# usnistgov/object-detection-yolov3

Measured on AMD Instinct MI355X. Metric: images/sec (train fwd+bwd) bs=8 416x416, higher is better.
Workload: dtype f32

## Files before the change

include/yolo3hip.h:

```cpp
#ifndef YOLO3HIP_H
#define YOLO3HIP_H

#include <math.h>
#include <stddef.h>
#include <stdint.h>

#ifdef __cplusplus
extern "C" {
#endif

#define Y3_OK 0
#define Y3_EINVAL (-1)
#define Y3_ELAUNCH (-2)

typedef void* y3_stream_t;

const char* y3_last_error(void);
int y3_debug_div(int x, int d);
int y3_version(void);

#define Y3_EPI_LRELU 1u
#define Y3_EPI_ACCUM 2u
#define Y3_CONV_X3 4u
int y3_x3_split_weights(const float* w, void* planes, int taps, int rows, int k_per_row, y3_stream_t stream);
// ... 1 lines not shown
int y3_x3_prepare_weights_batched(const float* params, float* params_t, void* planes, void* planes_t, const int* table_dev, int nlayers,
                                  int total_tiles, y3_stream_t stream);

typedef struct y3_tensor {
    float* ptr;
    int n, h, w, c;
    int ld;
} y3_tensor;

int y3_conv2d_fwd(const y3_tensor* src, const float* wt, const float* bias, int ksize, int stride,
                  const y3_tensor* dst, unsigned flags, float alpha,
                  const float* scale, const float* shift, const y3_tensor* resid,
                  float* stats, void* workspace, size_t workspace_bytes, y3_stream_t stream);
int y3_conv2d_stats_tiles(int m, int cin, int ksize, int cout);
size_t y3_conv2d_fwd_workspace(int m, int cin, int ksize, int cout);
int y3_conv2d_stats_tiles_x(int m, int cin, int ksize, int cout, unsigned flags);
size_t y3_conv2d_fwd_workspace_x(int m, int cin, int ksize, int cout, unsigned flags);
int y3_conv2d_x3_ok(int m, int c, int ntaps, int nout);
int y3_conv2d_dgrad_x3_ok(const y3_tensor* ddst, int ksize, int stride, const y3_tensor* dsrc);
size_t y3_conv2d_plan(int m, int cin, int ksize, int cout, int* out13);
size_t y3_conv2d_plan_x(int m, int cin, int ksize, int cout, unsigned flags, int* out13);

int y3_conv2d_dgrad(const y3_tensor* ddst, const float* wt_t, int ksize, int stride,
                    const y3_tensor* dsrc, unsigned flags, void* workspace, size_t workspace_bytes,
                    y3_stream_t stream);
size_t y3_conv2d_dgrad_workspace(const y3_tensor* ddst, int ksize, int stride, const y3_tensor* dsrc);
size_t y3_conv2d_dgrad_workspace_x(const y3_tensor* ddst, int ksize, int stride, const y3_tensor* dsrc, unsigned flags);
int y3_conv2d_dgrad_bn(const y3_tensor* ddst, const float* wt_t, int ksize, int stride, const y3_tensor* dsrc,
                       unsigned flags, const y3_tensor* bn_a, float* bn_partials,
                       void* workspace, size_t workspace_bytes, y3_stream_t stream);
int y3_conv2d_dgrad_bn_tiles(const y3_tensor* ddst, int ksize, int stride, const y3_tensor* dsrc);
int y3_conv2d_dgrad_bn_tiles_x(const y3_tensor* ddst, int ksize, int stride, const y3_tensor* dsrc, unsigned flags);
size_t y3_conv2d_dgrad_plan_x(const y3_tensor* ddst, int ksize, int stride, const y3_tensor* dsrc, unsigned flags, int* out51);

int y3_conv2d_wgrad(const y3_tensor* src, const y3_tensor* ddst, int ksize, int stride,
                    float* dw, void* workspace, size_t workspace_bytes, y3_stream_t stream);
size_t y3_conv2d_wgrad_workspace(const y3_tensor* src, const y3_tensor* ddst, int ksize, int stride);
int y3_conv2d_wgrad_x(const y3_tensor* src, const y3_tensor* ddst, int ksize, int stride,
                      float* dw, unsigned flags, void* workspace, size_t workspace_bytes, y3_stream_t stream);
size_t y3_conv2d_wgrad_workspace_x(const y3_tensor* src, const y3_tensor* ddst, int ksize, int stride, unsigned flags);
int y3_conv2d_wgrad_x3_ok(int m, int cin, int ksize, int cout);
size_t y3_conv2d_wgrad_plan(int m, int cin, int ksize, int cout, int* out8);
size_t y3_conv2d_wgrad_plan_x(int m, int cin, int ksize, int cout, unsigned flags, int* out8);

int y3_transpose_weights(const float* wt, float* wt_t, int taps, int cin, int cout, y3_stream_t stream);
int y3_transpose_weights_batched(const float* params, float* params_t, const int* table_dev, int nlayers,
                                 int total_tiles, y3_stream_t stream);

int y3_bn_stats_finalize(const float* stats, int tiles, int c, int count,
                         const float* gamma, const float* beta, float eps, float momentum,
                         float* moving_mean, float* moving_var,
                         float* save_mean, float* save_rstd, float* scale, float* shift,
                         y3_stream_t stream);
int y3_bn_fold_inference(const float* gamma, const float* beta, const float* moving_mean,
                         const float* moving_var, float eps, int c, float* scale, float* shift,
                         y3_stream_t stream);
int y3_bn_fold_inference_batched(const float* params, const float* moving, float* chan, const int* table_dev,
                                 int nlayers, float eps, y3_stream_t stream);
int y3_bn_apply(const y3_tensor* a, const float* scale, const float* shift, const y3_tensor* resid,
                const y3_tensor* y, y3_stream_t stream);
int y3_bn_bwd_stats(const y3_tensor* dy, const y3_tensor* a, const y3_tensor* dres, int dres_accumulate,
                    const float* gamma, const float* save_mean, const float* save_rstd, float alpha,
                    float* dgamma, float* dbeta, float* dbias, float* coef,
                    void* workspace, size_t workspace_bytes, y3_stream_t stream);
size_t y3_bn_bwd_workspace(int m, int c);
int y3_bn_bwd_apply(const y3_tensor* dy, const y3_tensor* a, const float* coef, float alpha,
// ... 277 lines not shown
```

object-detection-yolov3_amd/csrc/conv.hip:

```cpp
#include <stdlib.h>

#include <type_traits>
#include <utility>

#include "common.h"
#include "conv_plan.h"

template <int BM, int BN, int WM, int WN, int BK>
__global__ __launch_bounds__(64 * WM * WN) void conv_igemm_kernel(const ConvArgs p) {
    constexpr int THREADS = 64 * WM * WN;
    constexpr int LDA = BK + 4;
    constexpr int TM = BM / WM, TN = BN / WN, MB = TM / 32, NB = TN / 32;
    constexpr int KV = BK / 4;
    constexpr int A_TOTAL = BM * KV, A_LOADS = (A_TOTAL + THREADS - 1) / THREADS;
    constexpr int BN4 = BN / 4;
    constexpr int B_TOTAL = BK * BN4, B_LOADS = (B_TOTAL + THREADS - 1) / THREADS;
    static_assert(THREADS % KV == 0 && TM % 32 == 0 && TN % 32 == 0, "tile shape");

    __shared__ __attribute__((aligned(16))) float As[2][BM * LDA];
    __shared__ __attribute__((aligned(16))) float Bs[2][BK * BN];
    __shared__ float red[2][WM][BN];

    const int tid = threadIdx.x, lane = tid & 63, wave = tid >> 6;
    const int l31 = lane & 31, lh = lane >> 5;
// ... 1075 lines not shown
        a.nb_fast = a.nbn;
        a.dv_nb = y3_make_div(a.nbn);
        set_split(a, q);
        a.sk_slab0 = 0;
        const bool split = q.s0 > 1;
        a.tickets = split ? (int*)workspace + tick : nullptr;
        a.slab = split ? (float*)((char*)workspace + Y3_WS_HEADER) + slab_floats : nullptr;
        if (split) {
            tick += q.tiles;
            slab_floats += (size_t)q.tiles * q.s0 * t.bm * t.bn;
        }
        a.bn_row0 = rows;
        rows += a.nbm;
        m.first[c] = first;
        first += q.tiles * q.s0;
    }
    for (int c = ncls; c <= 4; ++c) m.first[c] = first;
    const bool bns = cls[0].bn_a != nullptr;
    if (cls[0].x3) {
        if (pl.ws > 0)
            if (int e = check_tickets("conv2d_dgrad (stride 2, x3)", workspace, st)) return e;
        if (!y3_x3_multi_launch(m, t.bn, bns, first, st)) {
            y3_set_error("conv2d_dgrad: no merged x3 kernel for tile %dx%d", t.bm, t.bn);
            return Y3_EINVAL;
        }
    } else if (!(bns ? launch_fast_multi<true>(t, m, first, st) : launch_fast_multi<false>(t, m, first, st))) {
        y3_set_error("conv2d_dgrad: no merged kernel for tile %dx%d", t.bm, t.bn);
        return Y3_EINVAL;
    }
    Y3_CHECK_LAUNCH("conv_igemm_fast_multi");
    return Y3_OK;
}

static int issue_dgrad(DgradDesc& d, const y3_tensor* ddst, const float* wt_t, const y3_tensor* dsrc, const y3_tensor* bn_a, float* bn_partials,
                       void* workspace, size_t workspace_bytes, hipStream_t st) {
    for (int c = 0; c < d.ncls; ++c) {
        ConvArgs& p = d.cls[c];
        p.src = ddst->ptr;
        p.wt = wt_t;
        p.dst = dsrc->ptr;
        if (bn_a) {
            p.bn_a = bn_a->ptr;
            p.bn_a_ld = bn_a->ld;
            p.bn_part = bn_partials;
        }
    }
    if (d.how == DGRAD_MERGED_F32 || d.how == DGRAD_MERGED_X3) return launch_dgrad_multi(d.cls, d.ncls, d.multi, workspace, workspace_bytes, st);
    for (int c = 0; c < d.ncls; ++c)
        if (int e = launch_igemm(d.cls[c], d.g[c], workspace, workspace_bytes, st)) return e;
    return Y3_OK;
}

static int check_dgrad_args(const y3_tensor* ddst, const float* wt_t, int ksize, int stride, const y3_tensor* dsrc, unsigned flags) {
    if (int e = check_tensor(ddst, "conv2d_dgrad ddst")) return e;
    if (int e = check_tensor(dsrc, "conv2d_dgrad dsrc")) return e;
    Y3_CHECK_ARG(wt_t, "conv2d_dgrad: null weights");
    Y3_CHECK_ARG((flags & ~(Y3_EPI_ACCUM | Y3_CONV_X3)) == 0, "conv2d_dgrad: only Y3_EPI_ACCUM and Y3_CONV_X3 allowed");
    Y3_CHECK_ARG(!(flags & Y3_CONV_X3) || dgrad_x3(flags, ddst, ksize, stride, dsrc), "conv2d_dgrad: Y3_CONV_X3 does not take this shape (ask y3_conv2d_dgrad_x3_ok())");
    return Y3_OK;
}
extern "C" int y3_conv2d_dgrad(const y3_tensor* ddst, const float* wt_t, int ksize, int stride, const y3_tensor* dsrc, unsigned flags,
                               void* workspace, size_t workspace_bytes, y3_stream_t stream) {
    if (int e = check_dgrad_args(ddst, wt_t, ksize, stride, dsrc, flags)) return e;
    DgradDesc d;
    if (int e = describe_dgrad(ddst, ksize, stride, dsrc, flags, &d)) return e;
    return issue_dgrad(d, ddst, wt_t, dsrc, nullptr, nullptr, workspace, workspace_bytes, (hipStream_t)stream);
}
extern "C" int y3_conv2d_dgrad_bn(const y3_tensor* ddst, const float* wt_t, int ksize, int stride, const y3_tensor* dsrc, unsigned flags,
                                  const y3_tensor* bn_a, float* bn_partials, void* workspace, size_t workspace_bytes, y3_stream_t stream) {
    if (int e = check_tensor(bn_a, "conv2d_dgrad_bn bn_a")) return e;
    Y3_CHECK_ARG(bn_partials, "conv2d_dgrad_bn: null partials");
    Y3_CHECK_ARG(dsrc && bn_a->n == dsrc->n && bn_a->h == dsrc->h && bn_a->w == dsrc->w && bn_a->c == dsrc->c, "conv2d_dgrad_bn: bn_a must have dsrc's geometry");
    Y3_CHECK_ARG((long long)bn_a->n * bn_a->h * bn_a->w * bn_a->ld * 4 < 0x7fffffffLL, "conv2d_dgrad_bn: bn_a of 2 GiB or more");
    DgradDesc d;
    Y3_CHECK_ARG(ddst && describe_dgrad(ddst, ksize, stride, dsrc, flags, &d) == Y3_OK && d.rows > 0, "conv2d_dgrad_bn: shape does not qualify (y3_conv2d_dgrad_bn_tiles() == 0)");
    if (int e = check_dgrad_args(ddst, wt_t, ksize, stride, dsrc, flags)) return e;
    return issue_dgrad(d, ddst, wt_t, dsrc, bn_a, bn_partials, workspace, workspace_bytes, (hipStream_t)stream);
}

extern "C" int y3_conv2d_wgrad(const y3_tensor* src, const y3_tensor* ddst, int ksize, int stride, float* dw, void* workspace,
                               size_t workspace_bytes, y3_stream_t stream) {
    return y3_conv2d_wgrad_x(src, ddst, ksize, stride, dw, 0u, workspace, workspace_bytes, stream);
}

extern "C" int y3_conv2d_wgrad_x(const y3_tensor* src, const y3_tensor* ddst, int ksize, int stride, float* dw, unsigned flags, void* workspace,
                                 size_t workspace_bytes, y3_stream_t stream) {
    if (int e = check_tensor(src, "conv2d_wgrad src")) return e;
    if (int e = check_tensor(ddst, "conv2d_wgrad ddst")) return e;
    Y3_CHECK_ARG(dw, "conv2d_wgrad: null dw");
    Y3_CHECK_ARG(ksize == 1 || ksize == 3, "conv2d_wgrad: ksize %d unsupported", ksize);
    Y3_CHECK_ARG(stride == 1 || stride == 2, "conv2d_wgrad: stride %d unsupported", stride);
    Y3_CHECK_ARG((src->c & 3) == 0, "conv2d_wgrad: Cin=%d must be a multiple of 4", src->c);
    const int OH = (src->h + stride - 1) / stride, OW = (src->w + stride - 1) / stride;
    Y3_CHECK_ARG(ddst->n == src->n && ddst->h == OH && ddst->w == OW, "conv2d_wgrad: geometry mismatch");
    WgradArgs p = {};
    const int taps = ksize * ksize;
    if (int e = set_channels(src->c, taps, &p.logC, &p.cmask)) return e;
    const int pbh = y3_same_pad_before(src->h, ksize, stride), pbw = y3_same_pad_before(src->w, ksize, stride);
    for (int kh = 0; kh < ksize; ++kh)
        for (int kw = 0; kw < ksize; ++kw) {
            const int t = kh * ksize + kw;
            p.tap_dhdw |= (unsigned long long)((kh - pbh + 1) | ((kw - pbw + 1) << 2)) << (4 * t);
        }
    p.src = src->ptr;
    p.ddst = ddst->ptr;
    p.H = src->h;
    p.W = src->w;
    p.C = src->c;
    p.src_ld = src->ld;
    p.OH = OH;
// ... 78 lines not shown
```

object-detection-yolov3_amd/csrc/conv_plan.cpp:

```cpp
#include <stdlib.h>
#include "host.h"
#include "conv_plan.h"

static TileCfg pick_tile(int M, int Nout) {
    TileCfg t;
    if (Nout <= 32)
        t = {128, 32, 16};
    else if (Nout <= 64)
        t = {128, 64, 16};
    else {
        const long long t128 = (long long)y3_cdiv(M, 128) * y3_cdiv(Nout, 128);
        const long long t64x128 = (long long)y3_cdiv(M, 64) * y3_cdiv(Nout, 128);
        if (t128 >= 600)
            t = {128, 128, 16};
        else if (t64x128 >= 600)
            t = {64, 128, 16};
        else
            t = {64, 64, 16};
    }
    return t;
}
void whole_tiles(ConvPlan& pl, int chunk) {
    pl.f = pl.tiles;
    pl.s0 = pl.s1 = 1;
// ... 262 lines not shown
        for (int c = 0; c < ncls; ++c) {
            const int sc = y3_cdiv(steps[c], L);
            if (sc > 1) {
                ConvPlan& q = pl->c[c];
                q.chunk0 = q.chunk1 = even_steps(y3_cdiv(steps[c], sc));
                q.s0 = q.s1 = y3_cdiv(steps[c], q.chunk0);
            }
        }
    }
    size_t slab = 0;
    for (int c = 0; c < ncls; ++c)
        if (pl->c[c].s0 > 1) slab += (size_t)pl->c[c].tiles * pl->c[c].s0 * t.bm * t.bn * 4;
    pl->ws = slab ? (size_t)Y3_WS_HEADER + slab : 0;
    return true;
}
static bool plan_dgrad_multi(const ConvArgs* cls, int ncls, MultiPlan* pl) {
    if (ncls < 2 || ncls > 4) return false;
    if (!(cls[0].x3 ? plan_dgrad_multi_x3(cls, ncls, pl) : plan_dgrad_multi_f32(cls, ncls, pl))) return false;
    FastGeom g;
    for (int c = 0; c < ncls; ++c)
        if (!fast_geom(cls[c], cls[c].K / cls[c].C, 16, &g)) return false;
    return true;
}

bool dgrad_x3(unsigned flags, const y3_tensor* ddst, int ksize, int stride, const y3_tensor* dsrc) {
    if (!(flags & Y3_CONV_X3) || !ddst || !dsrc) return false;
    if (stride == 1) return x3_shape_ok(ddst->c, dsrc->c, ksize * ksize * ddst->c, ksize * ksize);
    return stride == 2 && ksize == 3 && dsrc->c >= 64 && y3_is_pow2(ddst->c) && x3_shape_ok(ddst->c, dsrc->c, ddst->c, 1);
}
extern "C" int y3_conv2d_dgrad_x3_ok(const y3_tensor* ddst, int ksize, int stride, const y3_tensor* dsrc) {
    return dgrad_x3(Y3_CONV_X3, ddst, ksize, stride, dsrc) ? 1 : 0;
}

int describe_dgrad(const y3_tensor* ddst, int ksize, int stride, const y3_tensor* dsrc, unsigned flags, DgradDesc* d) {
    Y3_CHECK_ARG(ksize == 1 || ksize == 3, "conv2d_dgrad: ksize %d unsupported", ksize);
    Y3_CHECK_ARG(stride == 1 || stride == 2, "conv2d_dgrad: stride %d unsupported", stride);
    const int OH = (dsrc->h + stride - 1) / stride, OW = (dsrc->w + stride - 1) / stride;
    Y3_CHECK_ARG(ddst->n == dsrc->n && ddst->h == OH && ddst->w == OW, "conv2d_dgrad: geometry mismatch");
    const int pbh = y3_same_pad_before(dsrc->h, ksize, stride), pbw = y3_same_pad_before(dsrc->w, ksize, stride);
    ConvArgs base = {};
    base.H = ddst->h;
    base.W = ddst->w;
    base.C = ddst->c;
    base.src_ld = ddst->ld;
    base.dst_ld = dsrc->ld;
    base.Nout = dsrc->c;
    base.flags = flags & ~Y3_CONV_X3;
    base.x3 = dgrad_x3(flags, ddst, ksize, stride, dsrc) ? 1 : 0;
    base.DH = dsrc->h;
    base.DW = dsrc->w;
    base.sh = base.sw = 1;
    base.src_n = ddst->n;
    base.wt_rows = ksize * ksize * ddst->c;
    d->ncls = 0;
    d->rows = 0;
    d->ws_bytes = 0;
    if (stride == 1) {
        ConvArgs& p = d->cls[0];
        p = base;
        d->ncls = 1;
        const int taps = ksize * ksize;
        if (int e = set_channels(ddst->c, taps, &p.logC, &p.cmask)) return e;
        for (int kh = 0; kh < ksize; ++kh)
            for (int kw = 0; kw < ksize; ++kw) {
                const int t = kh * ksize + kw;
                const int dh = pbh - kh, dw = pbw - kw;
                p.tap_dhdw |= (unsigned long long)((dh + 1) | ((dw + 1) << 2)) << (4 * t);
                p.tap_wsel |= (unsigned long long)t << (4 * t);
            }
        p.OH = dsrc->h;
        p.OW = dsrc->w;
        p.dsh = p.dsw = 1;
        p.dense_dst = 1;
        p.K = taps * ddst->c;
        p.M = dsrc->n * p.OH * p.OW;
        d->how = DGRAD_SINGLE;
        d->g[0] = describe_gemm(p);
        d->ws_bytes = d->g[0].pl.ws_bytes;
// ... 26 lines not shown
            p.dense_dst = 0;
            p.M = dsrc->n * p.OH * p.OW;
            Y3_CHECK_ARG(nt > 0, "conv2d_dgrad: 1x1 stride-2 not supported");
            if (int e = set_channels(ddst->c, nt == 1 ? 1 : 9, &p.logC, &p.cmask)) return e;
            p.K = nt * ddst->c;
            cls[d->ncls++] = p;
        }
    for (int i = 1; i < d->ncls; ++i)
        for (int j = i; j > 0 && cls[j].K > cls[j - 1].K; --j) {
            const ConvArgs tmp = cls[j];
            cls[j] = cls[j - 1];
            cls[j - 1] = tmp;
        }
    if (plan_dgrad_multi(cls, d->ncls, &d->multi)) {
        d->how = base.x3 ? DGRAD_MERGED_X3 : DGRAD_MERGED_F32;
        d->rows = d->multi.rows;
        d->ws_bytes = d->multi.ws;
        return Y3_OK;
    }
    d->how = DGRAD_BY_CLASS;
    for (int c = 0; c < d->ncls; ++c) {
        d->g[c] = describe_gemm(cls[c]);
        if (d->g[c].pl.ws_bytes > d->ws_bytes) d->ws_bytes = d->g[c].pl.ws_bytes;
    }
    return Y3_OK;
}

extern "C" size_t y3_conv2d_dgrad_workspace(const y3_tensor* ddst, int ksize, int stride, const y3_tensor* dsrc) {
    return y3_conv2d_dgrad_workspace_x(ddst, ksize, stride, dsrc, 0u);
}
extern "C" size_t y3_conv2d_dgrad_workspace_x(const y3_tensor* ddst, int ksize, int stride, const y3_tensor* dsrc, unsigned flags) {
    if (stride == 1) return describe_gemm(dsrc->n * dsrc->h * dsrc->w, ddst->c, ksize * ksize, dsrc->c, flags).pl.ws_bytes;
    DgradDesc d;
    if (describe_dgrad(ddst, ksize, stride, dsrc, flags, &d) == Y3_OK && d.how == DGRAD_MERGED_X3) return d.ws_bytes;
    size_t best = 0;
    for (int nt = 1; nt <= 4; nt *= 2) {
        const size_t b = describe_gemm(dsrc->n * ((dsrc->h + 1) / 2) * ((dsrc->w + 1) / 2), ddst->c, nt, dsrc->c, 0u).pl.ws_bytes;
        if (b > best) best = b;
    }
    return best;
}

extern "C" int y3_conv2d_dgrad_bn_tiles(const y3_tensor* ddst, int ksize, int stride, const y3_tensor* dsrc) {
    return y3_conv2d_dgrad_bn_tiles_x(ddst, ksize, stride, dsrc, 0u);
}
extern "C" int y3_conv2d_dgrad_bn_tiles_x(const y3_tensor* ddst, int ksize, int stride, const y3_tensor* dsrc, unsigned flags) {
    DgradDesc d;
    return ddst && dsrc && describe_dgrad(ddst, ksize, stride, dsrc, flags, &d) == Y3_OK ? d.rows : 0;
}

extern "C" size_t y3_conv2d_dgrad_plan_x(const y3_tensor* ddst, int ksize, int stride, const y3_tensor* dsrc, unsigned flags, int* out51) {
    DgradDesc d;
    if (!ddst || !dsrc || describe_dgrad(ddst, ksize, stride, dsrc, flags, &d) != Y3_OK) {
        if (out51) out51[0] = -1;
        return 0;
    }
    if (out51) {
        for (int i = 0; i < 51; ++i) out51[i] = 0;
        out51[0] = (int)d.how;
        out51[1] = d.ncls;
        out51[2] = d.rows;
        const bool merged = d.how == DGRAD_MERGED_F32 || d.how == DGRAD_MERGED_X3;
        for (int c = 0; c < d.ncls; ++c) {
            const ConvPlan& pl = merged ? d.multi.c[c] : d.g[c].pl;
            const int fast = merged ? 1 : ((d.g[c].fast ? 1 : 0) | (pl.short_last ? 2 : 0));
            const int v[12] = {d.cls[c].K / d.cls[c].C, d.cls[c].M, pl.t.bm, pl.t.bn, pl.tiles, pl.f, pl.s0, pl.s1, pl.chunk0, pl.chunk1,
                               d.cls[c].K / pl.t.bk, fast};
            for (int i = 0; i < 12; ++i) out51[3 + 12 * c + i] = v[i];
        }
    }
    return d.ws_bytes;
}

static WgradPlan plan_wgrad(int K, int Nout, int M, int taps) {
    WgradPlan w;
    w.bkr = (K <= 64) ? 64 : 128;
    w.bn = (Nout <= 32) ? 32 : (Nout <= 64 ? 64 : 128);
    if (w.bkr == 128 && w.bn == 128) {
        if (taps == 1) {
            w.bkr = 64;
            w.bn = 64;
        } else if ((long long)K * Nout >= (1 << 20)) {
            w.bn = 64;
        } else if (K <= 576) {
            w.bkr = 64;
        }
// ... 77 lines not shown
```

object-detection-yolov3_amd/csrc/conv_plan.h:

```cpp
#pragma once
#include "host.h"

struct ConvArgs {
    const float* src;
    const float* wt;
    float* dst;
    const float* bias;
    const float* scale;
    const float* shift;
    const float* resid;
    float* stats;
    unsigned long long tap_dhdw;
    unsigned long long tap_wsel;
    int H, W, C, logC, cmask, src_ld;
    int OH, OW, sh, sw;
    int DH, DW, dsh, dsw, doh, dow, dst_ld, dense_dst;
    int resid_ld;
    int Nout, K, M;
    unsigned flags;
    float alpha;
    int nbn;
    int src_n, wt_rows;
    const float* bn_a;
    float* bn_part;
// ... 37 lines not shown

enum DgradHow {
    DGRAD_SINGLE,
    DGRAD_MERGED_F32,
    DGRAD_MERGED_X3,
    DGRAD_BY_CLASS
};
struct DgradDesc {
    ConvArgs cls[4];
    int ncls;
    DgradHow how;
    GemmDesc g[4];
    MultiPlan multi;
    int rows;
    size_t ws_bytes;
};

#define Y3_WG_FANIN 8
#define Y3_WG_TABLE 2048
struct WgradPlan {
    int bkr, bn, splits, chunk, tiles;
    bool x3;
    int grid;
    bool in_kernel;
    size_t ws_bytes;
};

void whole_tiles(ConvPlan& pl, int chunk);
bool no_room(size_t need, const void* workspace, size_t workspace_bytes);
bool fast_geom(const ConvArgs& a, int ntaps, int bk, FastGeom* g);
int set_channels(int C, int taps, int* logC, int* cmask);
GemmDesc describe_gemm(const ConvArgs& a);
bool dgrad_x3(unsigned flags, const y3_tensor* ddst, int ksize, int stride, const y3_tensor* dsrc);
int describe_dgrad(const y3_tensor* ddst, int ksize, int stride, const y3_tensor* dsrc, unsigned flags, DgradDesc* d);
WgradPlan describe_wgrad(int M, int cin, int taps, int Nout, unsigned flags);
```

object-detection-yolov3_amd/yolo3/_hip.py:

```python
import ctypes as C
import os

import torch

_HERE = os.path.dirname(os.path.abspath(__file__))
LIB_PATH = os.environ.get('Y3_LIB') or os.path.join(_HERE, '_lib', 'libyolo3hip.so')


class HipLibraryMissing(ImportError):
    pass


class HipError(RuntimeError):
    pass


if not os.path.exists(LIB_PATH):
    raise HipLibraryMissing(
        'libyolo3hip.so not found at %s: build it with `make -C object-detection-yolov3_amd/csrc` '
        '(hipcc --offload-arch=gfx950).  There is no CPU fallback.' % LIB_PATH)

lib = C.CDLL(LIB_PATH)


# ... 81 lines not shown
    'y3_loss_fwd_bwd_focal': (i32, [TP, fp, C.POINTER(C.c_float), i32, i32, i32, i32, f32, i32, f32, fp, ip, i32, f32, fp, fp, TP, vp, f32, f32, f32,
                                    f32, f32, vp]),
    'y3_adam_step': (i32, [fp, fp, fp, fp, sz, fp, f32, f32, f32, vp]),
    'y3_adam_step_ema': (i32, [fp, fp, fp, fp, sz, fp, f32, f32, f32, fp, fp, fp, sz, fp, vp]),
    'y3_grad_norm_workspace_bytes': (sz, [sz]),
    'y3_grad_accumulate': (i32, [fp, fp, sz, ip, vp, vp]),
    'y3_grad_sumsq': (i32, [fp, sz, vp, vp]),
    'y3_grad_clip_scale': (i32, [vp, sz, i32, C.c_double, fp, fp, vp]),
    'y3_adam_step_scaled': (i32, [fp, fp, fp, fp, sz, fp, f32, f32, f32, fp, vp]),
    'y3_adam_step_ema_scaled': (i32, [fp, fp, fp, fp, sz, fp, f32, f32, f32, fp, fp, fp, sz, fp, fp, vp]),
    'y3_optim_step': (i32, [C.POINTER(OptimDesc), vp]),
    'y3_nms_per_class': (i32, [fp, i32, i32, i32, f32, f32, f32, f32, f32, ip, ip, fp, i32, vp, sz, vp]),
    'y3_nms_workspace_bytes': (sz, [i32, i32, i32]),
    'y3_nms_single_class': (i32, [fp, i32, f32, ip, ip, fp, vp, sz, vp]),
    'y3_nms_per_class_ex': (i32, [fp, i32, i32, i32, i32, f32, f32, f32, f32, f32, f32, ip, ip, fp, i32, vp, sz, vp]),
    'y3_nms_workspace_bytes_ex': (sz, [i32, i32, i32, i32]),
    'y3_nms_labelled': (i32, [fp, i32, i32, i32, f32, f32, f32, ip, ip, fp, i32, vp, sz, vp]),
    'y3_tile_merge': (i32, [fp, i32, i32, i32, i32, ip, ip, fp, i32, ip, i32, i32, i32, i32, i32, f32, fp, i32, ip, vp, sz, vp]),
    'y3_tile_merge_workspace_bytes': (sz, [i32, i32]),
    'y3_tta_views_nhwc': (i32, [fp, i32, i32, i32, i32, C.POINTER(C.c_int), i32, TP, vp]),
    'y3_tta_unmap': (i32, [fp, i32, i32, i32, C.POINTER(C.c_int), i32, i32, i32, vp]),
    'y3_box_vote': (i32, [fp, i32, i32, i32, ip, ip, fp, i32, f32, f32, f32, f32, f32, i32, i32, i32, fp, vp, sz, vp]),
    'y3_box_vote_workspace_bytes': (sz, [i32, i32, i32]),
    'y3_filter_small_boxes': (i32, [fp, i32, i32, f32, ip, ip, vp]),
    'y3_compute_iou': (i32, [fp, fp, i32, i32, fp, vp]),
    'y3_comm_unique_id': (i32, [vp]),
    'y3_comm_init': (i32, [vp, i32, i32, C.POINTER(C.c_void_p)]),
    'y3_allreduce_sum_f32': (i32, [vp, fp, sz, vp]),
    'y3_conv2d_plan': (sz, [i32, i32, i32, i32, C.POINTER(C.c_int)]),
    'y3_conv2d_wgrad_plan': (sz, [i32, i32, i32, i32, C.POINTER(C.c_int)]),
    'y3_conv2d_plan_x': (sz, [i32, i32, i32, i32, u32, C.POINTER(C.c_int)]),
    'y3_conv2d_wgrad_plan_x': (sz, [i32, i32, i32, i32, u32, C.POINTER(C.c_int)]),
    'y3_conv2d_dgrad_plan_x': (sz, [TP, i32, i32, TP, u32, C.POINTER(C.c_int)]),
    'y3_comm_info': (i32, [vp, C.POINTER(C.c_int), C.POINTER(C.c_int)]),
    'y3_comm_destroy': (i32, [vp]),
    'y3_zscore': (i32, [fp, fp, i32, sz, vp, vp]),
    'y3_zscore_workspace_bytes': (sz, [i32]),
    'y3_augment_batch': (i32, [vp, i32, i32, i32, i32, i32, vp, i32, i32, fp, vp, vp]),
    'y3_augment_workspace_bytes': (sz, [i32, i32, i32, i32]),
    'y3_mosaic_batch': (i32, [fp, i32, i32, i32, i32, vp, fp, vp]),
    'y3_affine_batch': (i32, [fp, i32, i32, i32, i32, vp, fp, vp]),
    'y3_letterbox_batch': (i32, [vp, i32, i32, i32, vp, i32, i32, f32, fp, vp]),
    'y3_letterbox_zscore_nhwc': (i32, [vp, i32, i32, i32, vp, TP, vp, vp]),
    'y3_letterbox_workspace_bytes': (sz, [i32, i32, i32, i32]),
    'y3_letterbox_unmap': (i32, [fp, i32, i32, i32, vp, i32, vp]),
    'y3_format_labels': (i32, [ip, ip, i32, i32, C.POINTER(C.c_float), i32, i32, i32, i32, fp, fp, fp, vp]),
    'y3_anchor_stats_workspace_bytes': (sz, [i32, i32]),
    'y3_anchor_stats': (i32, [ip, C.c_longlong, fp, i32, i32, i32, i32, vp, vp, vp, vp]),
    'y3_eval_offsets':(i32, [ip, i32, i32, i32, ip, vp]),
    'y3_eval_match': (i32, [fp, i32, i32, i32, i32, f32, f32, ip, ip, fp, i32, i32, fp, ip, i32, i32, C.POINTER(C.c_float), i32, ip,
                            vp, vp, C.c_longlong, vp]),
    'y3_eval_ap': (i32, [vp, vp, C.c_longlong, i32, i32, ip, vp, sz, fp, fp, ip, ip, vp]),
    'y3_eval_ap_workspace_bytes': (sz, [C.c_longlong, i32]),
    'y3_eval_match_ranges': (i32, [fp, i32, i32, i32, i32, f32, f32, ip, ip, fp, i32, i32, fp, ip, i32, i32, C.POINTER(C.c_float), i32,
                                   C.POINTER(C.c_float), C.POINTER(C.c_float), i32, ip, vp, vp, vp, C.c_longlong, vp]),
    'y3_eval_ap_ranges': (i32, [vp, vp, vp, C.c_longlong, i32, i32, i32, ip, vp, sz, fp, fp, ip, ip, ip, ip, ip, fp, fp, fp, vp]),
    'y3_eval_ap_ranges_workspace_bytes': (sz, [C.c_longlong, i32, i32]),
}

for _name, (_res, _args) in SIGNATURES.items():
    _f = getattr(lib, _name)
    _f.restype = _res
    _f.argtypes = _args

EPI_LRELU = 1
EPI_ACCUM = 2
BF16_ROUTE_PP, BF16_ROUTE_C32, BF16_ROUTE_C64, BF16_ROUTE_RING = 1, 2, 3, 4
BF16_NO_PATCH = 8
OPT_SGD, OPT_SGD_NESTEROV, OPT_ADAMW, OPT_MAX_RANGES = 0, 1, 2, 128
CONV_X3 = 4


def check(rc, what=''):
    if rc != 0:
        raise HipError('%s failed (%d): %s' % (what or 'libyolo3hip call', rc, lib.y3_last_error().decode()))


def view(t, n, h, w, c, ld=None, offset=0):
    return Tensor(t.data_ptr() + t.element_size() * offset, n, h, w, c, c if ld is None else ld)


def float_array(vals):
    arr = (C.c_float * len(vals))(*[float(v) for v in vals])
    return arr


def int_array(vals):
    return (C.c_int * len(vals))(*[int(v) for v in vals])
```

object-detection-yolov3_amd/yolo3/model.py:

```python
import collections
import contextlib
import ctypes
import functools
import math
import os
import warnings

import numpy as np
import torch

from . import _hip
from . import letterbox
from . import streams
from ._hip import lib, check, view, int_array, EPI_LRELU, EPI_ACCUM, CONV_X3, BF16_NO_PATCH

BN_EPS = 1e-3
BN_MOMENTUM = 0.99
LRELU_ALPHA = 0.2
BF16_PATCH_MIN_BYTES = 300e6
ALIGN = 64


def ema_one_minus_decay(ema_decay, ema_warmup, t):
    d = float(ema_decay) * (1.0 - math.exp(-float(t) / float(ema_warmup)))
# ... 312 lines not shown
    def torch_view(self):
        flat = self.buf.view(-1)
        return torch.as_strided(flat, (self.n, self.h, self.w, self.c), (self.h * self.w * self.ld, self.w * self.ld, self.ld, 1), self.off)


class Mean:

    def __init__(self, name='mean', dtype=None):
        self.name = name
        self.reset_states()

    def update_state(self, value):
        self.total = self.total + (value.detach() if torch.is_tensor(value) else float(value))
        self.count += 1

    def result(self):
        if self.count == 0:
            return 0.0
        t = self.total / self.count
        return float(t.item()) if torch.is_tensor(t) else float(t)

    def reset_states(self):
        self.total = 0.0
        self.count = 0


def _pixels(v):
    return v.n * v.h * v.w


_WS_QUERY = {
    'y3_conv2d_fwd': lambda src, wt, bias, k, s, dst, flags, *_: lib.y3_conv2d_fwd_workspace_x(_pixels(dst), src.c, k, dst.c, flags),
    'y3_conv2d_fwd_bf16_ws': lambda src, wt, bias, k, s, dst, *_: lib.y3_conv2d_fwd_bf16_workspace(_pixels(dst), src.c, k, dst.c),
    'y3_conv2d_dgrad': lambda ddst, wt, k, s, dsrc, flags: lib.y3_conv2d_dgrad_workspace_x(ddst, k, s, dsrc, flags),
    'y3_conv2d_dgrad_bn': lambda ddst, wt, k, s, dsrc, flags, *_: lib.y3_conv2d_dgrad_workspace_x(ddst, k, s, dsrc, flags),
}

_Layer = collections.namedtuple('_Layer', 'fwd dgrad wgrad bn')


class _Plan:

    def __init__(self, model, n, training, bf16, size):
        self.model = model
        self.size = size
        self.n = n
        self.training = training
        self.bf16 = bool(bf16) and not training
        self.fwd = []
        self.bwd = []
        self.keep = []
        self.tensors = []
        self.graph = None
        self.graph_micro = None
        self.infer_graph = None
        self.infer_graph_tiles = None
        self.zs_ws = None
        self.lb_ws = None
        self._build()

    def _new(self, n, h, w, c, ld=None, zero=False, dtype=torch.float32):
        ld = c if ld is None else ld
        numel = n * h * w * ld
        buf = (torch.zeros if zero else torch.empty)(numel, dtype=dtype, device=self.model.device)
        t = _T(buf, n, h, w, c, ld)
        self.tensors.append(t)
        return t
# ... 240 lines not shown
                                                                 BOX_LOSSES.index(mdl.box_loss), mdl.box_loss_weight,
                                                                 self.loss4.data_ptr(), f.grad.v, ws)))
            f.gw = True
        if tr:
            self._build_backward()
        self._bind_conv_workspace()

    def _grad_of(self, t):
        if t.grad is None:
            if t.parent is not None:
                self._grad_of(t.parent)
                return t.grad
            t.grad = self._new(t.n, t.h, t.w, t.c, t.ld)
            for ch in t.children:
                ch.grad = _T(t.grad.buf, ch.n, ch.h, ch.w, ch.c, ch.ld, ch.off)
        return t.grad

    def _kernel_grad(self, fn, *args):
        args += (self.wg_ws.data_ptr(), self.wg_ws_bytes)
        if self.side is None:
            self._emit(self.bwd, fn, *args)
            return None
        self.events += [torch.cuda.Event(), torch.cuda.Event()]
        e_go, e_wg = len(self.events) - 2, len(self.events) - 1
        self.bwd.append(('record', e_go))
        self.keep.append(args)
        self.bwd.append(('side_call', (fn, args, e_go, e_wg)))
        return e_wg

    def _main_wait(self, e):
        if e is not None:
            self.bwd.append(('main_wait', e))

    def _build_backward(self):
        mdl = self.model
        specs = mdl.specs
        gptr = functools.partial(self._at, mdl.grads)

        wg_need = 0
        for op in self.ops:
            if op[0] in ('conv_layer', 'head'):
                sp = specs[op[1]]
                wg_need = max(wg_need, int(lib.y3_conv2d_wgrad_workspace_x(op[2].v, op[3].v, sp.k, sp.s, op[-1].wgrad)))
        self.wg_ws = torch.zeros(max(wg_need // 4, 4), dtype=torch.float32, device=mdl.device)
        self.wg_ws_bytes = wg_need

        epi_of = {}
        epi_for = {}
        first_consumer = {}
        for op in self.ops:
            reads = []
            if op[0] == 'conv_layer':
                reads = [op[2]] + ([op[5]] if op[5] is not None else [])
            elif op[0] == 'head':
                reads = [op[2]]
            elif op[0] in ('upsample', 'spp'):
                reads = [op[1]]
            for t in reads:
                first_consumer.setdefault(id(t), op)
                if t.parent is not None:
                    first_consumer.setdefault(id(t.parent), op)
                for ch in t.children:
                    first_consumer.setdefault(id(ch), op)
        for op in self.ops:
            if op[0] != 'conv_layer' or mdl.freeze_bn:
                continue
            a, y = op[3], op[4]
            cons = first_consumer.get(id(y))
            if cons is None or cons[0] != 'conv_layer' or cons[2] is not y or y.children or y is self.x0:
                continue
            csp = specs[cons[1]]
            tiles = int(lib.y3_conv2d_dgrad_bn_tiles_x(cons[3].v, csp.k, csp.s, y.v, cons[-1].dgrad))
            if tiles <= 0:
                continue
            part = torch.empty(tiles * 6 * y.c, dtype=torch.float32, device=mdl.device)
            epi_of[id(cons)] = (a, part, tiles)
            epi_for[id(op)] = (part, tiles)
        self.epilogue_stats_layers = len(epi_for)
        two = (not mdl.use_graph) and os.environ.get('Y3_WGRAD_STREAM', '1') != '0'
        self.side = streams.reserve(mdl.device)[0] if two else None
        self.events = []
        dz_bufs = [self.dz, torch.empty_like(self.dz)] if two else [self.dz]
        dz_busy = [None, None]
        head_wg = None
        nconv = 0
        for op in reversed(self.ops):
            kind = op[0]
            if kind == 'head':
                _, i, src, fm, _ = op
                sp = specs[i]
                dfm = fm.grad
                self._emit(self.bwd, lib.y3_colsum, dfm.v, gptr(sp.b_off))
                head_wg = self._kernel_grad(lib.y3_conv2d_wgrad, src.v, dfm.v, 1, 1, gptr(sp.w_off))
                if not src.no_grad:
                    ds = self._grad_of(src)
                    self._conv_call(self.bwd, lib.y3_conv2d_dgrad, dfm.v, self._at(mdl.params_t, sp.w_off), 1, 1, ds.v, EPI_ACCUM if src.gw else 0)
                    src.mark_written()
                self.bwd.append(('layer_done', i))
            elif kind == 'upsample':
                _, src, dst = op
                assert dst.gw and not src.gw
                ds = self._grad_of(src)
                self._emit(self.bwd, lib.y3_upsample_sum2x_bwd, dst.grad.v, ds.v)
                src.mark_written()
            elif kind == 'spp':
                _, src, cat, pools = op
                assert cat.gw and src.gw
                self._emit(self.bwd, lib.y3_spp_bwd, src.v, pools.grad.v, src.grad.v, 1)
            else:
                _, i, src, a, y, resid, x3 = op
                smean, srstd, coef = x3.bn
                sp = specs[i]
                assert y.gw, 'gradient of layer %d output never produced' % i
                dy = y.grad
                dr = None
                dr_acc = 0
                if resid is not None and not resid.no_grad:
                    dr = self._grad_of(resid)
                    dr_acc = 1 if resid.gw else 0
                    resid.mark_written()
                slot = nconv % len(dz_bufs)
                nconv += 1
                dz = _T(dz_bufs[slot], a.n, a.h, a.w, sp.cout)
                self.keep.append(dz)
                epi = epi_for.get(id(op))
                if mdl.freeze_bn:
                    assert int(lib.y3_bn_frozen_bwd_workspace(a.m, sp.cout)) <= self.bnb_ws.numel()
                    self._main_wait(dz_busy[slot])
                    self._emit(self.bwd, lib.y3_bn_frozen_bwd, dy.v, a.v, dr.v if dr is not None else None, dr_acc,
                               self._at(mdl.chan, sp.ch_off), self._at(mdl.moving, sp.mv_off), self._at(mdl.moving, mdl.moving_stride + sp.mv_off),
                               BN_EPS, LRELU_ALPHA, dz.v, gptr(sp.g_off), gptr(sp.be_off), gptr(sp.b_off), self.bnb_ws.data_ptr(), self.bnb_ws.numel())
                elif epi is not None:
                    part, tiles = epi
                    self._emit(self.bwd, lib.y3_bn_bwd_finalize_tiles, part.data_ptr(), tiles, sp.cout, a.m, self._at(mdl.params, sp.g_off),
                               smean, srstd, LRELU_ALPHA, gptr(sp.g_off), gptr(sp.be_off), gptr(sp.b_off), coef)
                else:
                    assert int(lib.y3_bn_bwd_workspace(a.m, sp.cout)) <= self.bnb_ws.numel()
                    self._emit(self.bwd, lib.y3_bn_bwd_stats, dy.v, a.v, dr.v if dr is not None else None, dr_acc,
                               self._at(mdl.params, sp.g_off), smean, srstd, LRELU_ALPHA, gptr(sp.g_off), gptr(sp.be_off), gptr(sp.b_off), coef,
                               self.bnb_ws.data_ptr(), self.bnb_ws.numel())
                if not mdl.freeze_bn:
                    self._main_wait(dz_busy[slot])
                    if epi is not None and dr is not None:
                        self._emit(self.bwd, lib.y3_bn_bwd_apply_fanin, dy.v, a.v, coef, LRELU_ALPHA, dz.v, dr.v, dr_acc)
                    else:
                        self._emit(self.bwd, lib.y3_bn_bwd_apply, dy.v, a.v, coef, LRELU_ALPHA, dz.v)
                dz_busy[slot] = self._kernel_grad(lib.y3_conv2d_wgrad_x, src.v, dz.v, sp.k, sp.s, gptr(sp.w_off), x3.wgrad)
                if x3.wgrad:
                    self.x3_wgrad.append(i)
                if not src.no_grad:
                    ds = self._grad_of(src)
                    wdg = self._at(mdl.planes, sp.w_off) if x3.dgrad else self._at(mdl.params_t, sp.w_off)
                    dflags = (EPI_ACCUM if src.gw else 0) | x3.dgrad
                    if x3.dgrad:
                        self.x3_dgrad.append(i)
                    if id(op) in epi_of:
                        pa, part, _ = epi_of[id(op)]
                        self._conv_call(self.bwd, lib.y3_conv2d_dgrad_bn, dz.v, wdg, sp.k, sp.s, ds.v, dflags, pa.v, part.data_ptr())
                        self.keep.append(part)
                    else:
                        self._conv_call(self.bwd, lib.y3_conv2d_dgrad, dz.v, wdg, sp.k, sp.s, ds.v, dflags)
                    src.mark_written()
                self.bwd.append(('layer_done', i))
        for e in dz_busy + [head_wg]:
            self._main_wait(e)

    def _run(self, lst, stream, dist=None):
        main = None
        pending = []
        for fn, args in lst:
            if fn == 'layer_done':
                if dist is not None:
                    if pending and dist.ends_bucket(args):
                        for e in pending:
                            main.wait_event(self.events[e])
                        pending = []
                    dist.on_layer_done(args)
                continue
            if fn in ('record', 'main_wait', 'side_call'):
                if main is None:
                    main = torch.cuda.current_stream(self.model.device)
                if fn == 'record':
                    self.events[args].record(main)
                elif fn == 'main_wait':
                    main.wait_event(self.events[args])
                else:
                    f2, a2, e_wait, e_done = args
                    self.side.wait_event(self.events[e_wait])
                    rc = f2(*a2, self.side.cuda_stream)
                    if rc != 0:
                        check(rc, f2.__name__)
                    self.events[e_done].record(self.side)
                    pending.append(e_done)
                continue
            rc = fn(*args, stream)
            if rc != 0:
# ... 832 lines not shown
```

Baseline: 559.0.

## Fold residual gradient fan-in into the dgrad epilogue of the consuming conv

```diff
diff --git a/include/yolo3hip.h b/include/yolo3hip.h
--- a/include/yolo3hip.h
+++ b/include/yolo3hip.h
@@ -57,6 +57,13 @@
 int y3_conv2d_dgrad_bn_tiles(const y3_tensor* ddst, int ksize, int stride, const y3_tensor* dsrc);
 int y3_conv2d_dgrad_bn_tiles_x(const y3_tensor* ddst, int ksize, int stride, const y3_tensor* dsrc, unsigned flags);
 size_t y3_conv2d_dgrad_plan_x(const y3_tensor* ddst, int ksize, int stride, const y3_tensor* dsrc, unsigned flags, int* out51);
+int y3_conv2d_dgrad_add(const y3_tensor* ddst, const float* wt_t, int ksize, int stride, const y3_tensor* dsrc, unsigned flags,
+                        const y3_tensor* dadd, void* workspace, size_t workspace_bytes, y3_stream_t stream);
+int y3_conv2d_dgrad_bn_add(const y3_tensor* ddst, const float* wt_t, int ksize, int stride, const y3_tensor* dsrc, unsigned flags,
+                           const y3_tensor* bn_a, float* bn_partials, const y3_tensor* dadd,
+                           void* workspace, size_t workspace_bytes, y3_stream_t stream);
+size_t y3_conv2d_dgrad_add_plan_x(const y3_tensor* ddst, int ksize, int stride, const y3_tensor* dsrc, const y3_tensor* dadd,
+                                  unsigned flags, int* out51);
 
 int y3_conv2d_wgrad(const y3_tensor* src, const y3_tensor* ddst, int ksize, int stride,
                     float* dw, void* workspace, size_t workspace_bytes, y3_stream_t stream);
diff --git a/object-detection-yolov3_amd/csrc/conv.hip b/object-detection-yolov3_amd/csrc/conv.hip
--- a/object-detection-yolov3_amd/csrc/conv.hip
+++ b/object-detection-yolov3_amd/csrc/conv.hip
@@ -1131,13 +1131,14 @@
     return Y3_OK;
 }
 
-static int issue_dgrad(DgradDesc& d, const y3_tensor* ddst, const float* wt_t, const y3_tensor* dsrc, const y3_tensor* bn_a, float* bn_partials,
-                       void* workspace, size_t workspace_bytes, hipStream_t st) {
+static int issue_dgrad(DgradDesc& d, const y3_tensor* ddst, const float* wt_t, const y3_tensor* dsrc, const y3_tensor* dadd, const y3_tensor* bn_a,
+                       float* bn_partials, void* workspace, size_t workspace_bytes, hipStream_t st) {
     for (int c = 0; c < d.ncls; ++c) {
         ConvArgs& p = d.cls[c];
         p.src = ddst->ptr;
         p.wt = wt_t;
         p.dst = dsrc->ptr;
+        p.resid = dadd ? dadd->ptr : nullptr;
         if (bn_a) {
             p.bn_a = bn_a->ptr;
             p.bn_a_ld = bn_a->ld;
@@ -1158,23 +1159,34 @@
     Y3_CHECK_ARG(!(flags & Y3_CONV_X3) || dgrad_x3(flags, ddst, ksize, stride, dsrc), "conv2d_dgrad: Y3_CONV_X3 does not take this shape (ask y3_conv2d_dgrad_x3_ok())");
     return Y3_OK;
 }
+extern "C" int y3_conv2d_dgrad_add(const y3_tensor* ddst, const float* wt_t, int ksize, int stride, const y3_tensor* dsrc, unsigned flags,
+                                   const y3_tensor* dadd, void* workspace, size_t workspace_bytes, y3_stream_t stream) {
+    if (int e = check_dgrad_args(ddst, wt_t, ksize, stride, dsrc, flags)) return e;
+    DgradDesc d;
+    if (int e = describe_dgrad(ddst, ksize, stride, dsrc, dadd, flags, &d)) return e;
+    return issue_dgrad(d, ddst, wt_t, dsrc, dadd, nullptr, nullptr, workspace, workspace_bytes, (hipStream_t)stream);
+}
 extern "C" int y3_conv2d_dgrad(const y3_tensor* ddst, const float* wt_t, int ksize, int stride, const y3_tensor* dsrc, unsigned flags,
                                void* workspace, size_t workspace_bytes, y3_stream_t stream) {
-    if (int e = check_dgrad_args(ddst, wt_t, ksize, stride, dsrc, flags)) return e;
-    DgradDesc d;
-    if (int e = describe_dgrad(ddst, ksize, stride, dsrc, flags, &d)) return e;
-    return issue_dgrad(d, ddst, wt_t, dsrc, nullptr, nullptr, workspace, workspace_bytes, (hipStream_t)stream);
-}
-extern "C" int y3_conv2d_dgrad_bn(const y3_tensor* ddst, const float* wt_t, int ksize, int stride, const y3_tensor* dsrc, unsigned flags,
-                                  const y3_tensor* bn_a, float* bn_partials, void* workspace, size_t workspace_bytes, y3_stream_t stream) {
+    return y3_conv2d_dgrad_add(ddst, wt_t, ksize, stride, dsrc, flags, nullptr, workspace, workspace_bytes, stream);
+}
+extern "C" int y3_conv2d_dgrad_bn_add(const y3_tensor* ddst, const float* wt_t, int ksize, int stride, const y3_tensor* dsrc, unsigned flags,
+                                      const y3_tensor* bn_a, float* bn_partials, const y3_tensor* dadd, void* workspace, size_t workspace_bytes,
+                                      y3_stream_t stream) {
     if (int e = check_tensor(bn_a, "conv2d_dgrad_bn bn_a")) return e;
     Y3_CHECK_ARG(bn_partials, "conv2d_dgrad_bn: null partials");
     Y3_CHECK_ARG(dsrc && bn_a->n == dsrc->n && bn_a->h == dsrc->h && bn_a->w == dsrc->w && bn_a->c == dsrc->c, "conv2d_dgrad_bn: bn_a must have dsrc's geometry");
     Y3_CHECK_ARG((long long)bn_a->n * bn_a->h * bn_a->w * bn_a->ld * 4 < 0x7fffffffLL, "conv2d_dgrad_bn: bn_a of 2 GiB or more");
     DgradDesc d;
-    Y3_CHECK_ARG(ddst && describe_dgrad(ddst, ksize, stride, dsrc, flags, &d) == Y3_OK && d.rows > 0, "conv2d_dgrad_bn: shape does not qualify (y3_conv2d_dgrad_bn_tiles() == 0)");
+    Y3_CHECK_ARG(ddst && describe_dgrad(ddst, ksize, stride, dsrc, nullptr, flags, &d) == Y3_OK && d.rows > 0, "conv2d_dgrad_bn: shape does not qualify (y3_conv2d_dgrad_bn_tiles() == 0)");
     if (int e = check_dgrad_args(ddst, wt_t, ksize, stride, dsrc, flags)) return e;
-    return issue_dgrad(d, ddst, wt_t, dsrc, bn_a, bn_partials, workspace, workspace_bytes, (hipStream_t)stream);
+    if (dadd)
+        if (int e = describe_dgrad(ddst, ksize, stride, dsrc, dadd, flags, &d)) return e;
+    return issue_dgrad(d, ddst, wt_t, dsrc, dadd, bn_a, bn_partials, workspace, workspace_bytes, (hipStream_t)stream);
+}
+extern "C" int y3_conv2d_dgrad_bn(const y3_tensor* ddst, const float* wt_t, int ksize, int stride, const y3_tensor* dsrc, unsigned flags,
+                                  const y3_tensor* bn_a, float* bn_partials, void* workspace, size_t workspace_bytes, y3_stream_t stream) {
+    return y3_conv2d_dgrad_bn_add(ddst, wt_t, ksize, stride, dsrc, flags, bn_a, bn_partials, nullptr, workspace, workspace_bytes, stream);
 }
 
 extern "C" int y3_conv2d_wgrad(const y3_tensor* src, const y3_tensor* ddst, int ksize, int stride, float* dw, void* workspace,
diff --git a/object-detection-yolov3_amd/csrc/conv_plan.cpp b/object-detection-yolov3_amd/csrc/conv_plan.cpp
--- a/object-detection-yolov3_amd/csrc/conv_plan.cpp
+++ b/object-detection-yolov3_amd/csrc/conv_plan.cpp
@@ -318,9 +318,25 @@
     return dgrad_x3(Y3_CONV_X3, ddst, ksize, stride, dsrc) ? 1 : 0;
 }
 
-int describe_dgrad(const y3_tensor* ddst, int ksize, int stride, const y3_tensor* dsrc, unsigned flags, DgradDesc* d) {
+static int check_dgrad_addend(int stride, const y3_tensor* dsrc, const y3_tensor* dadd, unsigned flags) {
+    Y3_CHECK_ARG(stride == 1, "conv2d_dgrad_add: an addend needs stride 1 (the parity classes of stride 2 have no dense destination)");
+    Y3_CHECK_ARG(!(flags & Y3_EPI_ACCUM), "conv2d_dgrad_add: Y3_EPI_ACCUM and an addend exclude each other");
+    Y3_CHECK_ARG(dadd->ptr && ((uintptr_t)dadd->ptr & 3) == 0 && dadd->c > 0 && (dadd->c & 3) == 0 && dadd->ld >= dadd->c,
+                 "conv2d_dgrad_add: dadd needs a 4-byte aligned pointer, c a multiple of 4 and ld >= c (c=%d ld=%d)", dadd->c, dadd->ld);
+    Y3_CHECK_ARG(dadd->n == dsrc->n && dadd->h == dsrc->h && dadd->w == dsrc->w && dadd->c == dsrc->c, "conv2d_dgrad_add: dadd must have dsrc's geometry");
+    const long long pix = (long long)dsrc->n * dsrc->h * dsrc->w;
+    Y3_CHECK_ARG(pix * dadd->ld * 4 < 0x7fffffffLL, "conv2d_dgrad_add: dadd of 2 GiB or more");
+    const uintptr_t al = (uintptr_t)dadd->ptr, ah = al + (uintptr_t)(((pix - 1) * dadd->ld + dadd->c) * 4);
+    const uintptr_t sl = (uintptr_t)dsrc->ptr, sh = sl + (uintptr_t)(((pix - 1) * dsrc->ld + dsrc->c) * 4);
+    Y3_CHECK_ARG(!(al < sh && sl < ah), "conv2d_dgrad_add: dadd overlaps dsrc");
+    return Y3_OK;
+}
+
+int describe_dgrad(const y3_tensor* ddst, int ksize, int stride, const y3_tensor* dsrc, const y3_tensor* dadd, unsigned flags, DgradDesc* d) {
     Y3_CHECK_ARG(ksize == 1 || ksize == 3, "conv2d_dgrad: ksize %d unsupported", ksize);
     Y3_CHECK_ARG(stride == 1 || stride == 2, "conv2d_dgrad: stride %d unsupported", stride);
+    if (dadd)
+        if (int e = check_dgrad_addend(stride, dsrc, dadd, flags)) return e;
     const int OH = (dsrc->h + stride - 1) / stride, OW = (dsrc->w + stride - 1) / stride;
     Y3_CHECK_ARG(ddst->n == dsrc->n && ddst->h == OH && ddst->w == OW, "conv2d_dgrad: geometry mismatch");
     const int pbh = y3_same_pad_before(dsrc->h, ksize, stride), pbw = y3_same_pad_before(dsrc->w, ksize, stride);
@@ -330,6 +346,7 @@
     base.C = ddst->c;
     base.src_ld = ddst->ld;
     base.dst_ld = dsrc->ld;
+    base.resid_ld = dadd ? dadd->ld : 0;
     base.Nout = dsrc->c;
     base.flags = flags & ~Y3_CONV_X3;
     base.x3 = dgrad_x3(flags, ddst, ksize, stride, dsrc) ? 1 : 0;
@@ -422,7 +439,7 @@
 extern "C" size_t y3_conv2d_dgrad_workspace_x(const y3_tensor* ddst, int ksize, int stride, const y3_tensor* dsrc, unsigned flags) {
     if (stride == 1) return describe_gemm(dsrc->n * dsrc->h * dsrc->w, ddst->c, ksize * ksize, dsrc->c, flags).pl.ws_bytes;
     DgradDesc d;
-    if (describe_dgrad(ddst, ksize, stride, dsrc, flags, &d) == Y3_OK && d.how == DGRAD_MERGED_X3) return d.ws_bytes;
+    if (describe_dgrad(ddst, ksize, stride, dsrc, nullptr, flags, &d) == Y3_OK && d.how == DGRAD_MERGED_X3) return d.ws_bytes;
     size_t best = 0;
     for (int nt = 1; nt <= 4; nt *= 2) {
         const size_t b = describe_gemm(dsrc->n * ((dsrc->h + 1) / 2) * ((dsrc->w + 1) / 2), ddst->c, nt, dsrc->c, 0u).pl.ws_bytes;
@@ -436,12 +453,16 @@
 }
 extern "C" int y3_conv2d_dgrad_bn_tiles_x(const y3_tensor* ddst, int ksize, int stride, const y3_tensor* dsrc, unsigned flags) {
     DgradDesc d;
-    return ddst && dsrc && describe_dgrad(ddst, ksize, stride, dsrc, flags, &d) == Y3_OK ? d.rows : 0;
+    return ddst && dsrc && describe_dgrad(ddst, ksize, stride, dsrc, nullptr, flags, &d) == Y3_OK ? d.rows : 0;
 }
 
 extern "C" size_t y3_conv2d_dgrad_plan_x(const y3_tensor* ddst, int ksize, int stride, const y3_tensor* dsrc, unsigned flags, int* out51) {
+    return y3_conv2d_dgrad_add_plan_x(ddst, ksize, stride, dsrc, nullptr, flags, out51);
+}
+extern "C" size_t y3_conv2d_dgrad_add_plan_x(const y3_tensor* ddst, int ksize, int stride, const y3_tensor* dsrc, const y3_tensor* dadd, unsigned flags,
+                                             int* out51) {
     DgradDesc d;
-    if (!ddst || !dsrc || describe_dgrad(ddst, ksize, stride, dsrc, flags, &d) != Y3_OK) {
+    if (!ddst || !dsrc || describe_dgrad(ddst, ksize, stride, dsrc, dadd, flags, &d) != Y3_OK) {
         if (out51) out51[0] = -1;
         return 0;
     }
diff --git a/object-detection-yolov3_amd/csrc/conv_plan.h b/object-detection-yolov3_amd/csrc/conv_plan.h
--- a/object-detection-yolov3_amd/csrc/conv_plan.h
+++ b/object-detection-yolov3_amd/csrc/conv_plan.h
@@ -93,5 +93,5 @@
 int set_channels(int C, int taps, int* logC, int* cmask);
 GemmDesc describe_gemm(const ConvArgs& a);
 bool dgrad_x3(unsigned flags, const y3_tensor* ddst, int ksize, int stride, const y3_tensor* dsrc);
-int describe_dgrad(const y3_tensor* ddst, int ksize, int stride, const y3_tensor* dsrc, unsigned flags, DgradDesc* d);
+int describe_dgrad(const y3_tensor* ddst, int ksize, int stride, const y3_tensor* dsrc, const y3_tensor* dadd, unsigned flags, DgradDesc* d);
 WgradPlan describe_wgrad(int M, int cin, int taps, int Nout, unsigned flags);
diff --git a/object-detection-yolov3_amd/yolo3/_hip.py b/object-detection-yolov3_amd/yolo3/_hip.py
--- a/object-detection-yolov3_amd/yolo3/_hip.py
+++ b/object-detection-yolov3_amd/yolo3/_hip.py
@@ -137,6 +137,9 @@
     'y3_conv2d_plan_x': (sz, [i32, i32, i32, i32, u32, C.POINTER(C.c_int)]),
     'y3_conv2d_wgrad_plan_x': (sz, [i32, i32, i32, i32, u32, C.POINTER(C.c_int)]),
     'y3_conv2d_dgrad_plan_x': (sz, [TP, i32, i32, TP, u32, C.POINTER(C.c_int)]),
+    'y3_conv2d_dgrad_add': (i32, [TP, fp, i32, i32, TP, u32, TP, vp, sz, vp]),
+    'y3_conv2d_dgrad_bn_add': (i32, [TP, fp, i32, i32, TP, u32, TP, fp, TP, vp, sz, vp]),
+    'y3_conv2d_dgrad_add_plan_x': (sz, [TP, i32, i32, TP, TP, u32, C.POINTER(C.c_int)]),
     'y3_comm_info': (i32, [vp, C.POINTER(C.c_int), C.POINTER(C.c_int)]),
     'y3_comm_destroy': (i32, [vp]),
     'y3_zscore': (i32, [fp, fp, i32, sz, vp, vp]),
@@ -168,6 +171,9 @@
     _f.restype = _res
     _f.argtypes = _args
 
+lib.y3_conv2d_dgrad_add.__name__ = 'y3_conv2d_dgrad'
+lib.y3_conv2d_dgrad_bn_add.__name__ = 'y3_conv2d_dgrad_bn'
+
 EPI_LRELU = 1
 EPI_ACCUM = 2
 BF16_ROUTE_PP, BF16_ROUTE_C32, BF16_ROUTE_C64, BF16_ROUTE_RING = 1, 2, 3, 4
diff --git a/object-detection-yolov3_amd/yolo3/model.py b/object-detection-yolov3_amd/yolo3/model.py
--- a/object-detection-yolov3_amd/yolo3/model.py
+++ b/object-detection-yolov3_amd/yolo3/model.py
@@ -368,7 +368,7 @@
 _WS_QUERY = {
     'y3_conv2d_fwd': lambda src, wt, bias, k, s, dst, flags, *_: lib.y3_conv2d_fwd_workspace_x(_pixels(dst), src.c, k, dst.c, flags),
     'y3_conv2d_fwd_bf16_ws': lambda src, wt, bias, k, s, dst, *_: lib.y3_conv2d_fwd_bf16_workspace(_pixels(dst), src.c, k, dst.c),
-    'y3_conv2d_dgrad': lambda ddst, wt, k, s, dsrc, flags: lib.y3_conv2d_dgrad_workspace_x(ddst, k, s, dsrc, flags),
+    'y3_conv2d_dgrad': lambda ddst, wt, k, s, dsrc, flags, *_: lib.y3_conv2d_dgrad_workspace_x(ddst, k, s, dsrc, flags),
     'y3_conv2d_dgrad_bn': lambda ddst, wt, k, s, dsrc, flags, *_: lib.y3_conv2d_dgrad_workspace_x(ddst, k, s, dsrc, flags),
 }
 
@@ -675,6 +675,32 @@
         if e is not None:
             self.bwd.append(('main_wait', e))
 
+    @staticmethod
+    def _grad_writer(op, t):
+        fam = [t] + ([t.parent] if t.parent is not None else []) + t.children
+        kind = op[0]
+        if kind == 'conv_layer':
+            if any(op[2] is f for f in fam) and not op[2].no_grad:
+                return 'src'
+            if op[5] is not None and any(op[5] is f for f in fam) and not op[5].no_grad:
+                return 'resid'
+            return None
+        src = op[2] if kind == 'head' else op[1]
+        return 'src' if any(src is f for f in fam) and not src.no_grad else None
+
+    def _fanin_in_epilogue(self, rops, k, resid, dy):
+        for op in rops[k + 1:]:
+            how = self._grad_writer(op, resid)
+            if how is None:
+                continue
+            if how != 'src' or op[0] != 'conv_layer' or op[2] is not resid:
+                return False
+            sp = self.model.specs[op[1]]
+            out51 = int_array([0] * 51)
+            lib.y3_conv2d_dgrad_add_plan_x(op[3].v, sp.k, sp.s, self._grad_of(resid).v, dy.v, op[-1].dgrad, out51)
+            return out51[0] >= 0
+        return False
+
     def _build_backward(self):
         mdl = self.model
         specs = mdl.specs
@@ -727,7 +753,11 @@
         dz_busy = [None, None]
         head_wg = None
         nconv = 0
-        for op in reversed(self.ops):
+        defer = os.environ.get('Y3_FANIN_PASS', '0') != '1'
+        addend = {}
+        self.fanin_deferred = 0
+        rops = list(reversed(self.ops))
+        for k, op in enumerate(rops):
             kind = op[0]
             if kind == 'head':
                 _, i, src, fm, _ = op
@@ -759,8 +789,12 @@
                 dr = None
                 dr_acc = 0
                 if resid is not None and not resid.no_grad:
-                    dr = self._grad_of(resid)
-                    dr_acc = 1 if resid.gw else 0
+                    if defer and not resid.gw and self._fanin_in_epilogue(rops, k, resid, dy):
+                        addend[id(resid)] = dy
+                        self.fanin_deferred += 1
+                    else:
+                        dr = self._grad_of(resid)
+                        dr_acc = 1 if resid.gw else 0
                     resid.mark_written()
                 slot = nconv % len(dz_bufs)
                 nconv += 1
@@ -794,17 +828,24 @@
                 if not src.no_grad:
                     ds = self._grad_of(src)
                     wdg = self._at(mdl.planes, sp.w_off) if x3.dgrad else self._at(mdl.params_t, sp.w_off)
-                    dflags = (EPI_ACCUM if src.gw else 0) | x3.dgrad
+                    dadd = addend.pop(id(src), None)
+                    dflags = (EPI_ACCUM if src.gw and dadd is None else 0) | x3.dgrad
                     if x3.dgrad:
                         self.x3_dgrad.append(i)
                     if id(op) in epi_of:
                         pa, part, _ = epi_of[id(op)]
-                        self._conv_call(self.bwd, lib.y3_conv2d_dgrad_bn, dz.v, wdg, sp.k, sp.s, ds.v, dflags, pa.v, part.data_ptr())
+                        if dadd is not None:
+                            self._conv_call(self.bwd, lib.y3_conv2d_dgrad_bn_add, dz.v, wdg, sp.k, sp.s, ds.v, dflags, pa.v, part.data_ptr(), dadd.v)
+                        else:
+                            self._conv_call(self.bwd, lib.y3_conv2d_dgrad_bn, dz.v, wdg, sp.k, sp.s, ds.v, dflags, pa.v, part.data_ptr())
                         self.keep.append(part)
+                    elif dadd is not None:
+                        self._conv_call(self.bwd, lib.y3_conv2d_dgrad_add, dz.v, wdg, sp.k, sp.s, ds.v, dflags, dadd.v)
                     else:
                         self._conv_call(self.bwd, lib.y3_conv2d_dgrad, dz.v, wdg, sp.k, sp.s, ds.v, dflags)
                     src.mark_written()
                 self.bwd.append(('layer_done', i))
+        assert not addend, 'a deferred residual fan-in was never added'
         for e in dz_busy + [head_wg]:
             self._main_wait(e)
 
```

Result: no change. 558.9, median of 2 (-0.0%).
